# srv902/FOCUS

Measured on AMD Instinct MI355X. Metric: clips/sec (fwd+bwd+opt step) ORViT-MF 16x224, higher is better.
Workload: dtype bf16; 1 GPU; ORViT-Motionformer 16x224, 4 objects, batch=8 per GPU (BASELINE configs[1]); global_batch=8, frames=16, crop=224, objects=4, parallelism=dp1, optimizer=adamw+clipnorm

## Files before the change

focus_amd/asm_lint.py:

```python
import re
import sys

_REG = re.compile(r"\b([va])(\d+)\b|\b([va])\[(\d+):(\d+)\]")
_VM_LOAD = re.compile(r"^(global_load|buffer_load|flat_load|scratch_load)_")
_EFFECT = re.compile(r"^(global_store|buffer_store|flat_store|scratch_store|ds_write|ds_store|global_atomic|buffer_atomic|flat_atomic|"
                     r"ds_add|ds_max|ds_min|ds_bpermute|ds_permute|v_cmp|v_cmpx|v_readlane|v_readfirstlane)")
_KEEPS = re.compile(r"fmac|_mac_|UNUSED_PRESERVE|op_sel|v_dot\w*c_|v_cvt_scalef32_pk_fp8|v_cvt_pk_fp8|v_cvt_sr_|sdwa|_dpp|v_writelane")
_SREG = re.compile(r"^s(\d+)$|^s\[(\d+):(\d+)\]$")


def _regs(text):
    regs = set()
    for m in _REG.finditer(text):
        if m.group(1) is not None:
            regs.add(int(m.group(2)) + (1000 if m.group(1) == "a" else 0))
        else:
            base = 1000 if m.group(3) == "a" else 0
            regs.update(range(base + int(m.group(4)), base + int(m.group(5)) + 1))
    return regs


def _srange(name):
    m = _SREG.match(name)
    if not m:
        return None
    return (int(m.group(1)),) * 2 if m.group(1) is not None else (int(m.group(2)), int(m.group(3)))


def _kernels(asm_path):
    out, name, body, in_asm, pending = [], None, [], False, None
    with open(asm_path) as f:
        for line in f:
            s = line.strip()
            if name is None:
                if pending is not None and s.startswith("; ScratchSize:"):
                    out.append((pending[0], pending[1], int(s.split(":")[1])))
                    pending = None
                m = re.match(r"^(_Z\w+):", line)
                if m:
                    name, body, in_asm = m.group(1), [], False
                continue
            if s.startswith(";;#ASMSTART"):
                in_asm = True
            elif s.startswith(";;#ASMEND"):
                in_asm = False
            elif s.startswith(".Lfunc_end"):
                pending, name = (name, body), None
            else:
                t = s.split(";", 1)[0].strip()
                if t:
                    body.append((t, in_asm))
    return out


def lint_kernel(body):
    labels = {t[:-1]: i for i, (t, _) in enumerate(body) if t.endswith(":")}
    problems, seen = set(), set()
    work = [(0, (), frozenset(), (), None, True)]
    while work:
        i, queue, poison, consts, vcc, live = work.pop()
        queue, poison, consts = list(queue), set(poison), dict(consts)
        while i < len(body):
            t, in_asm = body[i]
            if t.endswith(":"):
                while queue and not queue[0]:
                    queue.pop(0)
                key = (i, tuple(queue), frozenset(poison), tuple(sorted(consts.items())), vcc, live)
                if key in seen:
                    break
                seen.add(key)
                i += 1
                continue
            if t.startswith("."):
                i += 1
                continue
            parts = t.split(None, 1)
            op, args = parts[0], parts[1] if len(parts) > 1 else ""
            ops = [a.strip() for a in args.split(",")]
            if op == "s_waitcnt":
                m = re.search(r"vmcnt\((\d+)\)", t)
                if m:
                    del queue[:max(0, len(queue) - int(m.group(1)))]
                i += 1
                continue
            if op == "s_branch" or op.startswith("s_cbranch"):
                tgt = args.strip()
                if tgt in labels:
                    taken = {"s_cbranch_vccnz": vcc, "s_cbranch_vccz": None if vcc is None else 1 - vcc,
                             "s_cbranch_execnz": 1 if live else None, "s_cbranch_execz": 0 if live else None}.get(op)
                    if op == "s_branch" or taken == 1:
                        i = labels[tgt]
                        continue
                    if taken is None:
                        work.append((labels[tgt], tuple(queue), frozenset(poison), tuple(consts.items()), vcc, live))
                i += 1
                continue
            if op == "s_endpgm":
                break
            flying = frozenset().union(*queue) if queue else frozenset()
            dirty = flying | poison
            effect = bool(_EFFECT.match(op))
            dst = set() if effect and not op.startswith(("v_cmp", "v_read", "ds_bpermute", "ds_permute")) else _regs(ops[0] if ops else "")
            src = _regs(args) if not dst else _regs(",".join(ops[1:]))
            if op.startswith("v_swap"):
                src |= dst
            if dst & flying:
                problems.add("%s writes %s under a hand-issued load still in flight" % (op, _names(dst & flying)))
            hit = src & dirty
            sdst = bool(ops) and (ops[0].startswith(("s", "vcc", "exec", "m0")) and not ops[0].startswith("src"))
            if hit and (effect or sdst or _VM_LOAD.match(op)):
                problems.add("%s uses %s: %s" % (op, _names(hit), "loaded by hand and still in flight" if hit & flying else
                                                 "derived from a register read while its hand-issued load was in flight"))
            elif hit or (dst & poison and _KEEPS.search(t)):
                poison |= dst
            else:
                poison -= dst
            if _VM_LOAD.match(op):
                lds = "_lds_" in op or re.search(r"\blds\b", args)
                hand = in_asm and not lds
                queue.append(frozenset(dst) if hand else frozenset())
                poison -= dst
                if len(queue) > 96:
                    queue.pop(0)
            d0 = ops[0] if ops else ""
            if d0 == "exec" or "saveexec" in op:
                live = op.startswith("s_or_")
            if op == "s_and_b64" and d0 == "vcc" and "exec" in ops[1:] and any(o in consts for o in ops[1:]):
                vcc = 1 if consts[[o for o in ops[1:] if o in consts][0]] else 0
            else:
                if d0.startswith("vcc") or (op.startswith("v_cmp") and "_e64" not in op):
                    vcc = None
                r = _srange(d0)
                if r:
                    for k in [k for k in consts if _srange(k)[0] <= r[1] and r[0] <= _srange(k)[1]]:
                        del consts[k]
                    if op == "s_mov_b64" and len(ops) > 1 and ops[1] in ("-1", "0"):
                        consts[d0] = int(ops[1])
            i += 1
    return sorted(problems)


def _names(regs):
    return ",".join(("a%d" % (r - 1000)) if r >= 1000 else ("v%d" % r) for r in sorted(regs))


def lint_hand_loads(asm_path):
    problems = []
    for name, body, scratch in _kernels(asm_path):
        if not any(a and _VM_LOAD.match(t.split()[0]) for t, a in body if not t.endswith(":")):
            continue
        if scratch:
            problems.append((name, "scratch %d B/lane" % scratch))
        problems += [(name, p) for p in lint_kernel(body)]
    return problems


if __name__ == "__main__":
    for path in sys.argv[1:]:
        for p in lint_hand_loads(path):
            print("%s: %s" % p)
```

focus_amd/build.py:

```python
import concurrent.futures
import glob
import os
import re
import subprocess
import sys

HERE = os.path.dirname(os.path.abspath(__file__))
CSRC = os.path.join(HERE, "csrc")
OBJ = os.path.join(HERE, "lib", "obj")
LIB = os.path.join(HERE, "lib", "libfocus_amd.so")
HIPCC = os.environ.get("HIPCC", "/opt/rocm/bin/hipcc")
FLAGS = os.environ.get("FOCUS_EXTRA_HIPFLAGS", "").split() + ["--offload-arch=gfx950", "-O3", "-fPIC", "-std=c++17", "-Wno-pass-failed", "-Wall",
         "-Wno-unused-function"]


def _stale(target, deps):
    if not os.path.exists(target):
        return True
    t = os.path.getmtime(target)
    return any(os.path.getmtime(d) > t for d in deps)


def _hand_loads(src):
    with open(src) as f:
        return 'asm volatile("global_load_dword' in f.read()


def _device_asm(src):
    return os.path.join(OBJ, os.path.basename(src).replace(".hip", "-hip-amdgcn-amd-amdhsa-gfx950.s"))


def lint_hand_loads(asm_path):
    from focus_amd import asm_lint
    return asm_lint.lint_hand_loads(asm_path)


def _compile(src, headers):
    obj = os.path.join(OBJ, os.path.basename(src).replace(".hip", ".o"))
    if _stale(obj, [src] + headers):
        extra = ["-save-temps=obj"] if _hand_loads(src) else []
        subprocess.check_call([HIPCC] + FLAGS + extra + ["-c", src, "-o", obj])
    if _hand_loads(src):
        if not os.path.exists(_device_asm(src)):
            os.remove(obj)
            raise RuntimeError("%s issues loads by hand but its device assembly %s is missing: rebuild" % (
                os.path.basename(src), _device_asm(src)))
        bad = lint_hand_loads(_device_asm(src))
        if bad:
            os.remove(obj)
            raise RuntimeError("%s: registers of hand-issued loads touched before their wait (%d reports):\n  %s" % (
                os.path.basename(src), len(bad), "\n  ".join("%s: %s" % b for b in bad[:40])))
    return obj


def source_hash():
    import hashlib
    h = hashlib.sha1()
    for f in sorted(glob.glob(os.path.join(CSRC, "*.hip")) + glob.glob(os.path.join(CSRC, "*.h"))) + [
            os.path.join(HERE, "..", "include", "focus_amd.h")]:
        h.update(os.path.basename(f).encode())
        h.update(open(f, "rb").read())
    return h.hexdigest()[:12]


def _stamp():
    root = os.path.join(HERE, "..")
    head = "nogit"
    try:
        head = subprocess.run(["git", "-C", root, "rev-parse", "--short", "HEAD"], capture_output=True, text=True,
                              check=True).stdout.strip()
        if subprocess.run(["git", "-C", root, "status", "--porcelain", "--", "focus_amd/csrc", "include"],
                          capture_output=True, text=True).stdout.strip():
            head += "-dirty"
    except Exception:
        pass
    with open(os.path.join(HERE, "lib", "BUILD_HEAD"), "w") as f:
        f.write("%s src:%s\n" % (head, source_hash()))


def build(force=False, verbose=True):
    os.makedirs(OBJ, exist_ok=True)
    srcs = sorted(glob.glob(os.path.join(CSRC, "*.hip")))
    headers = sorted(glob.glob(os.path.join(CSRC, "*.h"))) + [os.path.join(HERE, "..", "include", "focus_amd.h")]
    if force:
        for f in glob.glob(os.path.join(OBJ, "*.o")):
            os.remove(f)
    with concurrent.futures.ThreadPoolExecutor(max_workers=min(8, len(srcs))) as ex:
        objs = list(ex.map(lambda s: _compile(s, headers), srcs))
    if _stale(LIB, objs):
        subprocess.check_call([HIPCC, "--offload-arch=gfx950", "-shared", "-fPIC", "-o", LIB] + objs)
    if os.path.isdir(os.path.join(HERE, "..", ".git")):
        _stamp()
    if verbose:
        print("built", LIB)
    return LIB


if __name__ == "__main__":
    build(force="--force" in sys.argv)
```

focus_amd/csrc/gemm_mfma_tn_ws.hip:

```cpp
#include "focus_common.h"
#include "gemm_internal.h"
#include <algorithm>
#include <cstdlib>

namespace {

typedef __attribute__((ext_vector_type(8))) __bf16 bf16x8;
typedef __attribute__((ext_vector_type(4))) short s16x4;
typedef __attribute__((ext_vector_type(4))) float f32x4;
typedef __attribute__((address_space(1))) const void gvoid_t;
typedef __attribute__((address_space(3))) void lvoid_t;
typedef __attribute__((address_space(3))) s16x4 lds_s16x4;

constexpr int BKM = 64;
constexpr int SUB = BKM * 256;
constexpr int NSTAGE = 3, NLOAD = 4;

union Frag { bf16x8 v; s16x4 t[2]; uint32_t u[4]; };

__device__ __forceinline__ int swz(int row) { return ((row & 3) | ((row >> 1) & 4)) << 1; }
__device__ __forceinline__ int toff(int row, int col) {
    return row * 256 + ((((col >> 3)) ^ swz(row)) << 4) + (col & 4) * 2;
}
__device__ __forceinline__ bf16x8 col_frag16(const char* tile, int r0, int c0, int lane) {
    const int i = lane & 15;
    const int row = r0 + (i >> 2), col = c0 + 4 * (i & 3);
    Frag f;
    f.t[0] = __builtin_amdgcn_ds_read_tr16_b64_v4i16((lds_s16x4*)(tile + toff(row, col)));
    f.t[1] = __builtin_amdgcn_ds_read_tr16_b64_v4i16((lds_s16x4*)(tile + toff(row + 4, col)));
    return f.v;
}

struct Unit { int i0, j0, m_begin, nk, valid_last; };

template <int BI, int BJ>
__global__ __launch_bounds__(64 * (BI * BJ / 4096 + NLOAD)) void gemm_tn_ws_kernel(const focus_gemm_desc d, int tiles_i, int tiles_j,
                                                                                  int splits, int m_per_split, float* csum) {
    constexpr int NCONS = BI * BJ / 4096;
    constexpr int WJ = BJ / 64;
    constexpr int NSP = BI / 128, NSQ = BJ / 128, NSUBT = NSP + NSQ;
    constexpr int STAGE = NSUBT * SUB;
    constexpr int PIECES = NSUBT * 16 / NLOAD;
    extern __shared__ __attribute__((aligned(16))) char smem[];

    const int tid = threadIdx.x, lane = tid & 63;
    const int w = __builtin_amdgcn_readfirstlane(tid >> 6);
    const int Mred = d.K;
    const bf16_t* Pm = static_cast<const bf16_t*>(d.A);
    const bf16_t* Qm = static_cast<const bf16_t*>(d.B);
    const int64_t ldp = d.csA, ldq = d.rsB;

    const int tiles = tiles_i * tiles_j, nunits = tiles * splits;
    const int G = gridDim.x, xcd = blockIdx.x & 7, jwg = blockIdx.x >> 3;
    const int gx = (G >> 3) + (xcd < (G & 7) ? 1 : 0);
    const int q = nunits >> 3, r = nunits & 7;
    const int band0 = xcd < r ? xcd * (q + 1) : r * (q + 1) + (xcd - r) * q;
    const int band_n = q + (xcd < r ? 1 : 0);
    const int my_units = jwg < band_n ? (band_n - jwg + gx - 1) / gx : 0;
    if (my_units == 0) return;
    auto unit_of = [&](int i) __attribute__((always_inline)) {
        const int u = band0 + jwg + i * gx;
        const int split = u / tiles, tile = u % tiles;
        Unit t;
        t.i0 = (tile % tiles_i) * BI;
        t.j0 = (tile / tiles_i) * BJ;
        t.m_begin = split * m_per_split;
        const int len = min(Mred, t.m_begin + m_per_split) - t.m_begin;
        t.nk = (len + BKM - 1) / BKM;
        t.valid_last = len - (t.nk - 1) * BKM;
        return t;
    };

    if (w >= NCONS) {
        const int L = w - NCONS;
        const int cpos = lane & 15, rin = lane >> 4;
        Unit cur = unit_of(0);
        int iu = 0, ikt = 0;
        auto issue = [&](int st) __attribute__((always_inline)) {
            char* sp = smem + st * STAGE;
            const int mb = cur.m_begin + ikt * BKM;
#pragma unroll
            for (int g = 0; g < PIECES; ++g) {
                const int sub = g >> 2, pi = g * NLOAD + L, row = (pi & 15) * 4 + rin;
                const int m = min(mb + row, Mred - 1);
                const int ch = cpos ^ swz(row);
                const bf16_t* src;
                if (sub < NSP) src = Pm + (int64_t)m * ldp + min(cur.i0 + sub * 128 + ch * 8, d.M - 8);
                else src = Qm + (int64_t)m * ldq + min(cur.j0 + (sub - NSP) * 128 + ch * 8, d.N - 8);
                __builtin_amdgcn_global_load_lds((gvoid_t*)src, (lvoid_t*)(sp + pi * 1024), 16, 0, 0);
            }
            if (++ikt == cur.nk) { ikt = 0; if (++iu < my_units) cur = unit_of(iu); }
        };
        int total = 0;
        for (int i = 0; i < my_units; ++i) total += unit_of(i).nk;
        issue(0);
        if (total > 1) {
            issue(1);
            asm volatile("s_waitcnt vmcnt(%0)" ::"n"(PIECES) : "memory");
        } else {
            asm volatile("s_waitcnt vmcnt(0)" ::: "memory");
        }
        __builtin_amdgcn_s_barrier();
        int st2 = 2;
        for (int t = 0; t < total; ++t) {
            if (t + 2 < total) {
                issue(st2);
                st2 = st2 == 2 ? 0 : st2 + 1;
                asm volatile("s_waitcnt vmcnt(%0)" ::"n"(PIECES) : "memory");
            } else {
                asm volatile("s_waitcnt vmcnt(0)" ::: "memory");
            }
            __builtin_amdgcn_s_barrier();
        }
        return;
    }

    const int wi = w / WJ, wj = w % WJ;
    const int fr = lane & 15, fq = lane >> 4;
    const int poff = (wi >> 1) * SUB, pcol = (wi & 1) * 64;
    const int qoff = (NSP + (wj >> 1)) * SUB, qcol = (wj & 1) * 64;
    f32x4 acc[4][4];
    constexpr int NA = 4 / WJ;
    f32x4 accb[NA];
    Frag ones;
    ones.u[0] = ones.u[1] = ones.u[2] = ones.u[3] = 0x3F803F80u;
    auto compute = [&](const char* stage, auto masked, int valid, bool cs) __attribute__((always_inline)) {
        const char* sp = stage + poff;
        const char* sq = stage + qoff;
#pragma unroll
        for (int ks = 0; ks < 2; ++ks) {
            bf16x8 fp[4], fqv[4];
#pragma unroll
            for (int a = 0; a < 4; ++a) fp[a] = col_frag16(sp, ks * 32 + 8 * fq, pcol + a * 16, lane);
#pragma unroll
            for (int b = 0; b < 4; ++b) fqv[b] = col_frag16(sq, ks * 32 + 8 * fq, qcol + b * 16, lane);
            if constexpr (decltype(masked)::value) {
                const int left = valid - (ks * 32 + 8 * fq);
#pragma unroll
                for (int a = 0; a < 4; ++a) {
                    Frag f; f.v = fp[a];
#pragma unroll
                    for (int e2 = 0; e2 < 4; ++e2) {
                        const uint32_t keep = (2 * e2 < left ? 0x0000ffffu : 0u) | (2 * e2 + 1 < left ? 0xffff0000u : 0u);
                        f.u[e2] &= keep;
                    }
                    fp[a] = f.v;
                }
            }
#pragma unroll
            for (int a = 0; a < 4; ++a)
#pragma unroll
                for (int b = 0; b < 4; ++b)
                    acc[a][b] = __builtin_amdgcn_mfma_f32_16x16x32_bf16(fqv[b], fp[a], acc[a][b], 0, 0, 0);
            if (cs) {
#pragma unroll
                for (int n = 0; n < NA; ++n) {
                    bf16x8 sel = fp[n];
#pragma unroll
                    for (int j = 1; j < WJ; ++j)
                        if (wj == j) sel = fp[j * NA + n];
                    accb[n] = __builtin_amdgcn_mfma_f32_16x16x32_bf16(ones.v, sel, accb[n], 0, 0, 0);
                }
            }
        }
    };

    __builtin_amdgcn_s_barrier();
    int st = 0;
    for (int cu = 0; cu < my_units; ++cu) {
        const Unit cur = unit_of(cu);
#pragma unroll
        for (int a = 0; a < 4; ++a)
#pragma unroll
            for (int b = 0; b < 4; ++b) acc[a][b] = (f32x4){0.f, 0.f, 0.f, 0.f};
        const int tj = cur.j0 / BJ;
        int cs_in = tj;
#pragma unroll
        for (int n = 0; n < NA; ++n) accb[n] = (f32x4){0.f, 0.f, 0.f, 0.f};
        for (int kt = 0; kt + 1 < cur.nk; ++kt) {
            compute(smem + st * STAGE, std::false_type{}, BKM, csum != nullptr && cs_in == 0);
            cs_in = cs_in == 0 ? tiles_j - 1 : cs_in - 1;
            st = st == 2 ? 0 : st + 1;
            __builtin_amdgcn_s_barrier();
        }
        compute(smem + st * STAGE, std::true_type{}, cur.valid_last, csum != nullptr && cs_in == 0);
        st = st == 2 ? 0 : st + 1;
        __builtin_amdgcn_s_barrier();
        const int split = cur.m_begin / m_per_split;
        if (csum && fq == 0) {
#pragma unroll
            for (int n = 0; n < NA; ++n) {
                const int gi = cur.i0 + wi * 64 + (wj * NA + n) * 16 + fr;
                if (gi < d.M) csum[(int64_t)(split * tiles_j + tj) * d.M + gi] = d.alpha * accb[n][0];
            }
        }
        float* C = d.aux ? static_cast<float*>(d.aux) + (int64_t)split * d.M * d.N : static_cast<float*>(d.C);
        const int64_t ldc = d.aux ? d.N : d.rsC;
#pragma unroll
        for (int a = 0; a < 4; ++a) {
            const int gi = cur.i0 + wi * 64 + a * 16 + fr;
            if (gi >= d.M) continue;
#pragma unroll
            for (int b = 0; b < 4; ++b) {
                const int gj = cur.j0 + wj * 64 + b * 16 + fq * 4;
                if (d.aux) {
                    if (gj < d.N)
                        *reinterpret_cast<float4*>(C + (int64_t)gi * ldc + gj) =
                            make_float4(d.alpha * acc[a][b][0], d.alpha * acc[a][b][1], d.alpha * acc[a][b][2], d.alpha * acc[a][b][3]);
                } else {
#pragma unroll
                    for (int r4 = 0; r4 < 4; ++r4)
                        if (gj + r4 < d.N) atomicAdd(C + (int64_t)gi * ldc + (gj + r4), d.alpha * acc[a][b][r4]);
                }
            }
        }
    }
}

template <int BI, int BJ>
int launch_tn_ws(const focus_gemm_desc& d, const focus_tn_plan& pl, float* csum, hipStream_t s) {
    const size_t lds = (size_t)NSTAGE * (BI / 128 + BJ / 128) * SUB;
    auto k = gemm_tn_ws_kernel<BI, BJ>;
    static bool once = (hipFuncSetAttribute((const void*)k, hipFuncAttributeMaxDynamicSharedMemorySize, lds) == hipSuccess);
    (void)once;
    const int nunits = pl.tiles_i * pl.tiles_j * pl.splits;
    hipLaunchKernelGGL(k, dim3(std::min(nunits, 256)), dim3(64 * (BI * BJ / 4096 + NLOAD)), lds, s, d, pl.tiles_i, pl.tiles_j,
                       pl.splits, pl.m_per_split, csum);
    FOCUS_CHECK_LAUNCH();
    return FOCUS_OK;
}

}

focus_tn_plan focus_gemm_tn_ws_plan(int M, int N, int K) {
    static const bool enabled = !(getenv("FOCUS_GEMM_TN_WS") && atoi(getenv("FOCUS_GEMM_TN_WS")) == 0);
    static const int rounds_env = getenv("FOCUS_GEMM_TN_ROUNDS") ? atoi(getenv("FOCUS_GEMM_TN_ROUNDS")) : 0;
    focus_tn_plan p = {};
    if (!enabled || M < 128 || N < 128 || K < 2048) return p;
    const int64_t pad1 = (int64_t)((M + 255) / 256 * 256) * ((N + 127) / 128 * 128);
    const int64_t pad2 = (int64_t)((M + 127) / 128 * 128) * ((N + 255) / 256 * 256);
    bool wide_i = (M >= N || N % 256 != 0) && M >= 256;
    static const bool pad_rule = !(getenv("FOCUS_GEMM_TN_PAD_RULE") && atoi(getenv("FOCUS_GEMM_TN_PAD_RULE")) == 0);
    if (wide_i && pad_rule && pad2 < pad1 && N < 256) wide_i = false;
    if (!wide_i && N < 256 && !(pad2 < pad1)) return p;
    const int bi = wide_i ? 256 : 128, bj = wide_i ? 128 : 256;
    p.kind = wide_i ? 1 : 2;
    p.tiles_i = (M + bi - 1) / bi;
    p.tiles_j = (N + bj - 1) / bj;
    const int tiles = p.tiles_i * p.tiles_j;
    const int max_splits = std::max(1, K / (4 * BKM));
    const int rounds = rounds_env > 0 ? rounds_env : 1;
    const int best_s = std::min(max_splits, std::max(1, 256 * rounds / tiles));
    p.splits = best_s;
    p.m_per_split = ((K + p.splits - 1) / p.splits + BKM - 1) / BKM * BKM;
    p.splits = (K + p.m_per_split - 1) / p.m_per_split;
    return p;
}

int focus_gemm_mfma_tn_ws(const focus_gemm_desc& d, const focus_tn_plan& pl, float* csum, hipStream_t s) {
    if (pl.kind == 1) return launch_tn_ws<256, 128>(d, pl, csum, s);
    if (pl.kind == 2) return launch_tn_ws<128, 256>(d, pl, csum, s);
    return FOCUS_ERR_SHAPE;
}
```

focus_amd/csrc/gemm_tn_group.hip:

```cpp
#include "focus_common.h"
#include "gemm_internal.h"
#include <algorithm>

namespace {

typedef __attribute__((ext_vector_type(8))) __bf16 bf16x8;
typedef __attribute__((ext_vector_type(4))) short s16x4;
typedef __attribute__((ext_vector_type(4))) float f32x4;
typedef __attribute__((address_space(1))) const void gvoid_t;
typedef __attribute__((address_space(3))) void lvoid_t;
typedef __attribute__((address_space(3))) s16x4 lds_s16x4;

constexpr int BKM = 64;
constexpr int SUB = BKM * 256;
constexpr int NSTAGE = 3, NLOAD = 4;
constexpr int BI = 256, BJ = 128;

union Frag { bf16x8 v; s16x4 t[2]; uint32_t u[4]; };

__device__ __forceinline__ int swz(int row) { return ((row & 3) | ((row >> 1) & 4)) << 1; }
__device__ __forceinline__ int toff(int row, int col) {
    return row * 256 + ((((col >> 3)) ^ swz(row)) << 4) + (col & 4) * 2;
}
__device__ __forceinline__ bf16x8 col_frag16(const char* tile, int r0, int c0, int lane) {
    const int i = lane & 15;
    const int row = r0 + (i >> 2), col = c0 + 4 * (i & 3);
    Frag f;
    f.t[0] = __builtin_amdgcn_ds_read_tr16_b64_v4i16((lds_s16x4*)(tile + toff(row, col)));
    f.t[1] = __builtin_amdgcn_ds_read_tr16_b64_v4i16((lds_s16x4*)(tile + toff(row + 4, col)));
    return f.v;
}

struct Prob {
    const bf16_t* P;
    const bf16_t* Q;
    float* C;
    float* db;
    int64_t ldp, ldq;
    int32_t I, J, Mred, tiles_i, tiles_j, pad_;
};
constexpr int MAXP = 8;
struct GroupArgs { Prob p[MAXP]; int32_t nprob, nunits; };
struct UnitRec { int16_t prob, ti, tj, pad_; };

__global__ __launch_bounds__(64 * (BI * BJ / 4096 + NLOAD)) void gemm_tn_group_kernel(const GroupArgs ga, const UnitRec* __restrict__ units) {
    constexpr int NCONS = BI * BJ / 4096;
    constexpr int WJ = BJ / 64;
    constexpr int NSP = BI / 128, NSQ = BJ / 128, NSUBT = NSP + NSQ;
    constexpr int STAGE = NSUBT * SUB;
    constexpr int PIECES = NSUBT * 16 / NLOAD;
    extern __shared__ __attribute__((aligned(16))) char smem[];

    const int tid = threadIdx.x, lane = tid & 63;
    const int w = __builtin_amdgcn_readfirstlane(tid >> 6);
    const int nunits = ga.nunits;
    const int G = gridDim.x, xcd = blockIdx.x & 7, jwg = blockIdx.x >> 3;
    const int gx = (G >> 3) + (xcd < (G & 7) ? 1 : 0);
    const int q8 = nunits >> 3, r8 = nunits & 7;
    const int band0 = xcd < r8 ? xcd * (q8 + 1) : r8 * (q8 + 1) + (xcd - r8) * q8;
    const int band_n = q8 + (xcd < r8 ? 1 : 0);
    const int my_units = jwg < band_n ? (band_n - jwg + gx - 1) / gx : 0;
    if (my_units == 0) return;

    struct Unit { const bf16_t* P; const bf16_t* Q; float* C; float* db; int64_t ldp, ldq; int I, J, Mred, i0, j0, nk, valid_last, tj; };
    auto unit_of = [&](int i) __attribute__((always_inline)) {
        const UnitRec ur = units[band0 + jwg + i * gx];
        const int pi = __builtin_amdgcn_readfirstlane((int)ur.prob);
        Unit t;
        Prob p = ga.p[0];
#pragma unroll
        for (int k = 1; k < MAXP; ++k)
            if (pi == k) p = ga.p[k];
        t.P = p.P; t.Q = p.Q; t.C = p.C; t.db = p.db; t.ldp = p.ldp; t.ldq = p.ldq; t.I = p.I; t.J = p.J; t.Mred = p.Mred;
        t.i0 = __builtin_amdgcn_readfirstlane((int)ur.ti) * BI;
        t.tj = __builtin_amdgcn_readfirstlane((int)ur.tj);
        t.j0 = t.tj * BJ;
        t.nk = (p.Mred + BKM - 1) / BKM;
        t.valid_last = p.Mred - (t.nk - 1) * BKM;
        return t;
    };

    if (w >= NCONS) {
        const int L = w - NCONS;
        const int cpos = lane & 15, rin = lane >> 4;
        Unit cur = unit_of(0);
        int iu = 0, ikt = 0;
        auto issue = [&](int st) __attribute__((always_inline)) {
            char* sp = smem + st * STAGE;
            const int mb = ikt * BKM;
#pragma unroll
            for (int g = 0; g < PIECES; ++g) {
                const int sub = g >> 2, pi = g * NLOAD + L, row = (pi & 15) * 4 + rin;
                const int m = min(mb + row, cur.Mred - 1);
                const int ch = cpos ^ swz(row);
                const bf16_t* src;
                if (sub < NSP) src = cur.P + (int64_t)m * cur.ldp + min(cur.i0 + sub * 128 + ch * 8, cur.I - 8);
                else src = cur.Q + (int64_t)m * cur.ldq + min(cur.j0 + (sub - NSP) * 128 + ch * 8, cur.J - 8);
                __builtin_amdgcn_global_load_lds((gvoid_t*)src, (lvoid_t*)(sp + pi * 1024), 16, 0, 0);
            }
            if (++ikt == cur.nk) { ikt = 0; if (++iu < my_units) cur = unit_of(iu); }
        };
        int total = 0;
        for (int i = 0; i < my_units; ++i) total += unit_of(i).nk;
        issue(0);
        if (total > 1) {
            issue(1);
            asm volatile("s_waitcnt vmcnt(%0)" ::"n"(PIECES) : "memory");
        } else {
            asm volatile("s_waitcnt vmcnt(0)" ::: "memory");
        }
        __builtin_amdgcn_s_barrier();
        int st2 = 2;
        for (int t = 0; t < total; ++t) {
            if (t + 2 < total) {
                issue(st2);
                st2 = st2 == 2 ? 0 : st2 + 1;
                asm volatile("s_waitcnt vmcnt(%0)" ::"n"(PIECES) : "memory");
            } else {
                asm volatile("s_waitcnt vmcnt(0)" ::: "memory");
            }
            __builtin_amdgcn_s_barrier();
        }
        return;
    }

    const int wi = w / WJ, wj = w % WJ;
    const int fr = lane & 15, fq = lane >> 4;
    const int poff = (wi >> 1) * SUB, pcol = (wi & 1) * 64;
    const int qoff = (NSP + (wj >> 1)) * SUB, qcol = (wj & 1) * 64;
    f32x4 acc[4][4];
    constexpr int NA = 4 / WJ;
    f32x4 accb[NA];
    Frag ones;
    ones.u[0] = ones.u[1] = ones.u[2] = ones.u[3] = 0x3F803F80u;
    auto compute = [&](const char* stage, auto masked, int valid, bool cs) __attribute__((always_inline)) {
        const char* sp = stage + poff;
        const char* sq = stage + qoff;
#pragma unroll
        for (int ks = 0; ks < 2; ++ks) {
            bf16x8 fp[4], fqv[4];
#pragma unroll
            for (int a = 0; a < 4; ++a) fp[a] = col_frag16(sp, ks * 32 + 8 * fq, pcol + a * 16, lane);
#pragma unroll
            for (int b = 0; b < 4; ++b) fqv[b] = col_frag16(sq, ks * 32 + 8 * fq, qcol + b * 16, lane);
            if constexpr (decltype(masked)::value) {
                const int left = valid - (ks * 32 + 8 * fq);
#pragma unroll
                for (int a = 0; a < 4; ++a) {
                    Frag f; f.v = fp[a];
#pragma unroll
                    for (int e2 = 0; e2 < 4; ++e2) {
                        const uint32_t keep = (2 * e2 < left ? 0x0000ffffu : 0u) | (2 * e2 + 1 < left ? 0xffff0000u : 0u);
                        f.u[e2] &= keep;
                    }
                    fp[a] = f.v;
                }
            }
#pragma unroll
            for (int a = 0; a < 4; ++a)
#pragma unroll
                for (int b = 0; b < 4; ++b)
                    acc[a][b] = __builtin_amdgcn_mfma_f32_16x16x32_bf16(fqv[b], fp[a], acc[a][b], 0, 0, 0);
            if (cs) {
#pragma unroll
                for (int n = 0; n < NA; ++n) {
                    bf16x8 sel = fp[n];
#pragma unroll
                    for (int j = 1; j < WJ; ++j)
                        if (wj == j) sel = fp[j * NA + n];
                    accb[n] = __builtin_amdgcn_mfma_f32_16x16x32_bf16(ones.v, sel, accb[n], 0, 0, 0);
                }
            }
        }
    };

    __builtin_amdgcn_s_barrier();
    int st = 0;
    for (int cu = 0; cu < my_units; ++cu) {
        const Unit cur = unit_of(cu);
#pragma unroll
        for (int a = 0; a < 4; ++a)
#pragma unroll
            for (int b = 0; b < 4; ++b) acc[a][b] = (f32x4){0.f, 0.f, 0.f, 0.f};
        const bool want_b = cur.db != nullptr && cur.tj == 0;
#pragma unroll
        for (int n = 0; n < NA; ++n) accb[n] = (f32x4){0.f, 0.f, 0.f, 0.f};
        for (int kt = 0; kt + 1 < cur.nk; ++kt) {
            compute(smem + st * STAGE, std::false_type{}, BKM, want_b);
            st = st == 2 ? 0 : st + 1;
            __builtin_amdgcn_s_barrier();
        }
        compute(smem + st * STAGE, std::true_type{}, cur.valid_last, want_b);
        st = st == 2 ? 0 : st + 1;
        __builtin_amdgcn_s_barrier();
        if (want_b && fq == 0) {
#pragma unroll
            for (int n = 0; n < NA; ++n) {
                const int gi = cur.i0 + wi * 64 + (wj * NA + n) * 16 + fr;
                if (gi < cur.I) cur.db[gi] = accb[n][0];
            }
        }
#pragma unroll
        for (int a = 0; a < 4; ++a) {
            const int gi = cur.i0 + wi * 64 + a * 16 + fr;
            if (gi >= cur.I) continue;
#pragma unroll
            for (int b = 0; b < 4; ++b) {
                const int gj = cur.j0 + wj * 64 + b * 16 + fq * 4;
                if (gj < cur.J)
                    *reinterpret_cast<float4*>(cur.C + (int64_t)gi * cur.J + gj) =
                        make_float4(acc[a][b][0], acc[a][b][1], acc[a][b][2], acc[a][b][3]);
            }
        }
    }
}

}

extern "C" int focus_linear_wgrad_group_units(const focus_wgrad_item* items, int n_items) {
    if (!items || n_items <= 0) return 0;
    int64_t t = 0;
    for (int p = 0; p < n_items; ++p) t += (int64_t)((items[p].N + BI - 1) / BI) * ((items[p].K + BJ - 1) / BJ);
    return t > 0x7fffffff ? -1 : (int)t;
}

extern "C" int focus_linear_wgrad_group_plan(const focus_wgrad_item* items, int n_items, void* host_units, size_t bytes) {
    if (!items || !host_units) return FOCUS_ERR_NULL;
    if (n_items <= 0 || n_items > MAXP) return FOCUS_ERR_SHAPE;
    const int total = focus_linear_wgrad_group_units(items, n_items);
    if (total <= 0 || bytes < (size_t)total * sizeof(UnitRec)) return FOCUS_ERR_WORKSPACE;
    UnitRec* u = static_cast<UnitRec*>(host_units);
    constexpr int BA = 4, BB = 8;
    int n = 0;
    for (int p = 0; p < n_items; ++p) {
        const int ti_n = (items[p].N + BI - 1) / BI, tj_n = (items[p].K + BJ - 1) / BJ;
        for (int bi = 0; bi < ti_n; bi += BA)
            for (int bj = 0; bj < tj_n; bj += BB)
                for (int ti = bi; ti < std::min(bi + BA, ti_n); ++ti)
                    for (int tj = bj; tj < std::min(bj + BB, tj_n); ++tj)
                        u[n++] = UnitRec{(int16_t)p, (int16_t)ti, (int16_t)tj, 0};
    }
    return n == total ? FOCUS_OK : FOCUS_ERR_SHAPE;
}

extern "C" int focus_linear_wgrad_group(const focus_wgrad_item* items, int n_items, const void* dev_units, void* stream) {
    if (!items || !dev_units) return FOCUS_ERR_NULL;
    if (n_items <= 0) return FOCUS_OK;
    if (n_items > MAXP) return FOCUS_ERR_SHAPE;
    GroupArgs ga = {};
    int units = 0;
    for (int p = 0; p < n_items; ++p) {
        const focus_wgrad_item& it = items[p];
        if (!it.dy || !it.x || !it.dw) return FOCUS_ERR_NULL;
        if (it.M <= 0 || it.N < 8 || it.K < 8 || (it.N & 7) || (it.K & 7) || (it.ld_dy & 7) || (it.ld_x & 7)) return FOCUS_ERR_SHAPE;
        if (!focus_aligned(it.dy, 16) || !focus_aligned(it.x, 16) || !focus_aligned(it.dw, 16)) return FOCUS_ERR_ALIGN;
        Prob& q = ga.p[p];
        q.P = static_cast<const bf16_t*>(it.dy); q.Q = static_cast<const bf16_t*>(it.x);
        q.C = it.dw; q.db = it.db; q.ldp = it.ld_dy; q.ldq = it.ld_x;
        q.I = it.N; q.J = it.K; q.Mred = it.M;
        q.tiles_i = (it.N + BI - 1) / BI; q.tiles_j = (it.K + BJ - 1) / BJ; q.pad_ = 0;
        if (q.tiles_i > 32767 || q.tiles_j > 32767) return FOCUS_ERR_SHAPE;
        units += q.tiles_i * q.tiles_j;
    }
    ga.nprob = n_items;
    ga.nunits = units;
    hipStream_t s = static_cast<hipStream_t>(stream);
    const size_t lds = (size_t)NSTAGE * (BI / 128 + BJ / 128) * SUB;
    auto k = gemm_tn_group_kernel;
    static bool once = (hipFuncSetAttribute((const void*)k, hipFuncAttributeMaxDynamicSharedMemorySize, lds) == hipSuccess);
    (void)once;
    hipLaunchKernelGGL(k, dim3(std::min(units, 256)), dim3(64 * (BI * BJ / 4096 + NLOAD)), lds, s, ga,
                       static_cast<const UnitRec*>(dev_units));
    FOCUS_CHECK_LAUNCH();
    return FOCUS_OK;
}
```

Measured before the change: 287.3 clips/s.

## Precompute loader source pointers per unit and specialize TN GEMM k-loop on bias-sum

The producer warps in both TN GEMM kernels now compute per-piece source pointers once per work unit and advance them by a k-stride. Only the last k-step still uses clamped row arithmetic. This removes 64-bit multiplies and min clamps from every global_load_lds issue. The grouped kernel reads the problem table straight from the kernarg segment instead of a select chain over MAXP entries. The consumer k-loop is split into two compile-time variants on whether the column-sum MFMA is needed, and an explicit lgkmcnt wait is added before each barrier. A new asm lint fails the build if vector integer multiplies remain beside the DMA loads outside the marked last step. The costs are extra live pointer registers in the loader and a duplicated k-loop body.

After: 297.6 clips/s (median of 6 runs). 1.04x the previous value.

```diff
diff --git a/focus_amd/asm_lint.py b/focus_amd/asm_lint.py
--- a/focus_amd/asm_lint.py
+++ b/focus_amd/asm_lint.py
@@ -155,7 +155,72 @@
     return problems
 
 
+TN_KERNELS = ("gemm_tn_group_kernel", "gemm_tn_ws_kernel")
+TN_MARKER = "focus-lint: clamped-last-step"
+_VMUL = re.compile(r"^(v_mul_lo_u32|v_mul_lo_i32|v_mul_hi_u32|v_mul_hi_i32|v_mad_u64_u32|v_mad_i64_i32)\b")
+_BLOCK_END = re.compile(r"^(s_branch|s_cbranch\w*|s_endpgm|s_setpc_b64)\b")
+
+
+def _raw_kernels(asm_path):
+    out, name, body, pending = [], None, [], None
+    with open(asm_path) as f:
+        for line in f:
+            s = line.strip()
+            if name is None:
+                if pending is not None and s.startswith("; ScratchSize:"):
+                    out.append((pending[0], pending[1], int(s.split(":")[1])))
+                    pending = None
+                m = re.match(r"^(_Z\w+):", line)
+                if m:
+                    name, body = m.group(1), []
+            elif s.startswith(".Lfunc_end"):
+                pending, name = (name, body), None
+            elif s:
+                body.append(s)
+    return out
+
+
+def lint_tn_loader(asm_path, kernels=TN_KERNELS):
+    problems, found = [], 0
+    for name, body, scratch in _raw_kernels(asm_path):
+        if not any(k in name for k in kernels):
+            continue
+        found += 1
+        if scratch:
+            problems.append((name, "scratch %d B/lane" % scratch))
+        blocks, cur = [], []
+        for s in body:
+            if re.match(r"^[.\w$]+:", s):
+                blocks.append(cur)
+                cur = []
+            cur.append(s)
+            if _BLOCK_END.match(s):
+                blocks.append(cur)
+                cur = []
+        blocks.append(cur)
+        dma = 0
+        for b in blocks:
+            code = [s.split(";", 1)[0].strip() for s in b]
+            loads = sum(c.startswith("global_load_lds_dwordx4") for c in code)
+            if not loads:
+                continue
+            dma += loads
+            muls = [c.split()[0] for c in code if _VMUL.match(c)]
+            if muls and not any(TN_MARKER in s for s in b):
+                label = b[0] if re.match(r"^[.\w$]+:", b[0]) else "(unlabelled)"
+                problems.append((name, "block %s issues %d global_load_lds_dwordx4 beside %d vector integer multiplies (%s)" % (
+                    label.split(":")[0], loads, len(muls), ",".join(sorted(set(muls))))))
+        if not dma:
+            problems.append((name, "no global_load_lds_dwordx4 found: the rule has nothing to check"))
+    if not found:
+        problems.append((asm_path, "none of the kernels %s found" % ", ".join(kernels)))
+    return problems
+
+
 if __name__ == "__main__":
     for path in sys.argv[1:]:
         for p in lint_hand_loads(path):
             print("%s: %s" % p)
+        if any(k in open(path).read() for k in TN_KERNELS):
+            for p in lint_tn_loader(path):
+                print("%s: %s" % p)
diff --git a/focus_amd/build.py b/focus_amd/build.py
--- a/focus_amd/build.py
+++ b/focus_amd/build.py
@@ -26,6 +26,13 @@
         return 'asm volatile("global_load_dword' in f.read()
 
 
+TN_LOADER_FILES = ("gemm_tn_group.hip", "gemm_mfma_tn_ws.hip")
+
+
+def _tn_loader(src):
+    return os.path.basename(src) in TN_LOADER_FILES
+
+
 def _device_asm(src):
     return os.path.join(OBJ, os.path.basename(src).replace(".hip", "-hip-amdgcn-amd-amdhsa-gfx950.s"))
 
@@ -35,11 +42,25 @@
     return asm_lint.lint_hand_loads(asm_path)
 
 
+def lint_tn_loader(asm_path):
+    from focus_amd import asm_lint
+    return asm_lint.lint_tn_loader(asm_path)
+
+
 def _compile(src, headers):
     obj = os.path.join(OBJ, os.path.basename(src).replace(".hip", ".o"))
     if _stale(obj, [src] + headers):
-        extra = ["-save-temps=obj"] if _hand_loads(src) else []
+        extra = ["-save-temps=obj"] if _hand_loads(src) or _tn_loader(src) else []
         subprocess.check_call([HIPCC] + FLAGS + extra + ["-c", src, "-o", obj])
+    if _tn_loader(src):
+        if not os.path.exists(_device_asm(src)):
+            os.remove(obj)
+            raise RuntimeError("%s: its device assembly %s is missing: rebuild" % (os.path.basename(src), _device_asm(src)))
+        bad = lint_tn_loader(_device_asm(src))
+        if bad:
+            os.remove(obj)
+            raise RuntimeError("%s: address arithmetic in the loader K loop or scratch use (%d reports):\n  %s" % (
+                os.path.basename(src), len(bad), "\n  ".join("%s: %s" % b for b in bad[:40])))
     if _hand_loads(src):
         if not os.path.exists(_device_asm(src)):
             os.remove(obj)
diff --git a/focus_amd/csrc/gemm_mfma_tn_ws.hip b/focus_amd/csrc/gemm_mfma_tn_ws.hip
--- a/focus_amd/csrc/gemm_mfma_tn_ws.hip
+++ b/focus_amd/csrc/gemm_mfma_tn_ws.hip
@@ -74,25 +74,43 @@
     if (w >= NCONS) {
         const int L = w - NCONS;
         const int cpos = lane & 15, rin = lane >> 4;
-        Unit cur = unit_of(0);
+        Unit cur;
+        const bf16_t* src[PIECES];
         int iu = 0, ikt = 0;
+        auto setup = [&](int i) __attribute__((always_inline)) {
+            cur = unit_of(i);
+#pragma unroll
+            for (int g = 0; g < PIECES; ++g) {
+                const int sub = g >> 2, pi = g * NLOAD + L, row = (pi & 15) * 4 + rin;
+                const int ch = cpos ^ swz(row);
+                if (sub < NSP) src[g] = Pm + (int64_t)(cur.m_begin + row) * ldp + min(cur.i0 + sub * 128 + ch * 8, d.M - 8);
+                else src[g] = Qm + (int64_t)(cur.m_begin + row) * ldq + min(cur.j0 + (sub - NSP) * 128 + ch * 8, d.N - 8);
+            }
+        };
         auto issue = [&](int st) __attribute__((always_inline)) {
             char* sp = smem + st * STAGE;
-            const int mb = cur.m_begin + ikt * BKM;
-#pragma unroll
-            for (int g = 0; g < PIECES; ++g) {
-                const int sub = g >> 2, pi = g * NLOAD + L, row = (pi & 15) * 4 + rin;
-                const int m = min(mb + row, Mred - 1);
-                const int ch = cpos ^ swz(row);
-                const bf16_t* src;
-                if (sub < NSP) src = Pm + (int64_t)m * ldp + min(cur.i0 + sub * 128 + ch * 8, d.M - 8);
-                else src = Qm + (int64_t)m * ldq + min(cur.j0 + (sub - NSP) * 128 + ch * 8, d.N - 8);
-                __builtin_amdgcn_global_load_lds((gvoid_t*)src, (lvoid_t*)(sp + pi * 1024), 16, 0, 0);
-            }
-            if (++ikt == cur.nk) { ikt = 0; if (++iu < my_units) cur = unit_of(iu); }
+            if (ikt + 1 < cur.nk) {
+                const int64_t kp = (int64_t)ikt * BKM * ldp, kq = (int64_t)ikt * BKM * ldq;
+#pragma unroll
+                for (int g = 0; g < PIECES; ++g)
+                    __builtin_amdgcn_global_load_lds((gvoid_t*)(src[g] + ((g >> 2) < NSP ? kp : kq)),
+                                                     (lvoid_t*)(sp + (g * NLOAD + L) * 1024), 16, 0, 0);
+            } else {
+                asm volatile("; focus-lint: clamped-last-step" ::: "memory");
+                const int mb = cur.m_begin + ikt * BKM;
+#pragma unroll
+                for (int g = 0; g < PIECES; ++g) {
+                    const int pi = g * NLOAD + L, row = (pi & 15) * 4 + rin;
+                    const int back = min(mb + row, Mred - 1) - (cur.m_begin + row);
+                    __builtin_amdgcn_global_load_lds((gvoid_t*)(src[g] + (int64_t)back * ((g >> 2) < NSP ? ldp : ldq)),
+                                                     (lvoid_t*)(sp + pi * 1024), 16, 0, 0);
+                }
+            }
+            if (++ikt == cur.nk) { ikt = 0; if (++iu < my_units) setup(iu); }
         };
         int total = 0;
         for (int i = 0; i < my_units; ++i) total += unit_of(i).nk;
+        setup(0);
         issue(0);
         if (total > 1) {
             issue(1);
@@ -124,7 +142,7 @@
     f32x4 accb[NA];
     Frag ones;
     ones.u[0] = ones.u[1] = ones.u[2] = ones.u[3] = 0x3F803F80u;
-    auto compute = [&](const char* stage, auto masked, int valid, bool cs) __attribute__((always_inline)) {
+    auto compute = [&](const char* stage, auto masked, int valid, auto has_cs, bool cs) __attribute__((always_inline)) {
         const char* sp = stage + poff;
         const char* sq = stage + qoff;
 #pragma unroll
@@ -152,7 +170,7 @@
 #pragma unroll
                 for (int b = 0; b < 4; ++b)
                     acc[a][b] = __builtin_amdgcn_mfma_f32_16x16x32_bf16(fqv[b], fp[a], acc[a][b], 0, 0, 0);
-            if (cs) {
+            if (decltype(has_cs)::value && cs) {
 #pragma unroll
                 for (int n = 0; n < NA; ++n) {
                     bf16x8 sel = fp[n];
@@ -177,15 +195,21 @@
         int cs_in = tj;
 #pragma unroll
         for (int n = 0; n < NA; ++n) accb[n] = (f32x4){0.f, 0.f, 0.f, 0.f};
-        for (int kt = 0; kt + 1 < cur.nk; ++kt) {
-            compute(smem + st * STAGE, std::false_type{}, BKM, csum != nullptr && cs_in == 0);
-            cs_in = cs_in == 0 ? tiles_j - 1 : cs_in - 1;
+        auto k_loop = [&](auto has_cs) __attribute__((always_inline)) {
+            for (int kt = 0; kt + 1 < cur.nk; ++kt) {
+                compute(smem + st * STAGE, std::false_type{}, BKM, has_cs, cs_in == 0);
+                cs_in = cs_in == 0 ? tiles_j - 1 : cs_in - 1;
+                st = st == 2 ? 0 : st + 1;
+                asm volatile("s_waitcnt lgkmcnt(0)" ::: "memory");
+                __builtin_amdgcn_s_barrier();
+            }
+            compute(smem + st * STAGE, std::true_type{}, cur.valid_last, has_cs, cs_in == 0);
             st = st == 2 ? 0 : st + 1;
+            asm volatile("s_waitcnt lgkmcnt(0)" ::: "memory");
             __builtin_amdgcn_s_barrier();
-        }
-        compute(smem + st * STAGE, std::true_type{}, cur.valid_last, csum != nullptr && cs_in == 0);
-        st = st == 2 ? 0 : st + 1;
-        __builtin_amdgcn_s_barrier();
+        };
+        if (csum) k_loop(std::true_type{});
+        else k_loop(std::false_type{});
         const int split = cur.m_begin / m_per_split;
         if (csum && fq == 0) {
 #pragma unroll
diff --git a/focus_amd/csrc/gemm_tn_group.hip b/focus_amd/csrc/gemm_tn_group.hip
--- a/focus_amd/csrc/gemm_tn_group.hip
+++ b/focus_amd/csrc/gemm_tn_group.hip
@@ -1,6 +1,7 @@
 #include "focus_common.h"
 #include "gemm_internal.h"
 #include <algorithm>
+#include <cstddef>
 
 namespace {
 
@@ -62,46 +63,63 @@
     const int my_units = jwg < band_n ? (band_n - jwg + gx - 1) / gx : 0;
     if (my_units == 0) return;
 
+    static_assert(offsetof(GroupArgs, p) == 0, "the problem table opens the kernel-argument segment");
+    typedef __attribute__((address_space(4))) const Prob cprob_t;
+    cprob_t* tab = (cprob_t*)__builtin_amdgcn_kernarg_segment_ptr();
     struct Unit { const bf16_t* P; const bf16_t* Q; float* C; float* db; int64_t ldp, ldq; int I, J, Mred, i0, j0, nk, valid_last, tj; };
     auto unit_of = [&](int i) __attribute__((always_inline)) {
         const UnitRec ur = units[band0 + jwg + i * gx];
-        const int pi = __builtin_amdgcn_readfirstlane((int)ur.prob);
+        cprob_t* p = tab + __builtin_amdgcn_readfirstlane((int)ur.prob);
         Unit t;
-        Prob p = ga.p[0];
-#pragma unroll
-        for (int k = 1; k < MAXP; ++k)
-            if (pi == k) p = ga.p[k];
-        t.P = p.P; t.Q = p.Q; t.C = p.C; t.db = p.db; t.ldp = p.ldp; t.ldq = p.ldq; t.I = p.I; t.J = p.J; t.Mred = p.Mred;
+        t.P = p->P; t.Q = p->Q; t.C = p->C; t.db = p->db; t.ldp = p->ldp; t.ldq = p->ldq; t.I = p->I; t.J = p->J; t.Mred = p->Mred;
         t.i0 = __builtin_amdgcn_readfirstlane((int)ur.ti) * BI;
         t.tj = __builtin_amdgcn_readfirstlane((int)ur.tj);
         t.j0 = t.tj * BJ;
-        t.nk = (p.Mred + BKM - 1) / BKM;
-        t.valid_last = p.Mred - (t.nk - 1) * BKM;
+        t.nk = (t.Mred + BKM - 1) / BKM;
+        t.valid_last = t.Mred - (t.nk - 1) * BKM;
         return t;
     };
 
     if (w >= NCONS) {
         const int L = w - NCONS;
         const int cpos = lane & 15, rin = lane >> 4;
-        Unit cur = unit_of(0);
+        Unit cur;
+        const bf16_t* src[PIECES];
         int iu = 0, ikt = 0;
+        auto setup = [&](int i) __attribute__((always_inline)) {
+            cur = unit_of(i);
+#pragma unroll
+            for (int g = 0; g < PIECES; ++g) {
+                const int sub = g >> 2, pi = g * NLOAD + L, row = (pi & 15) * 4 + rin;
+                const int ch = cpos ^ swz(row);
+                if (sub < NSP) src[g] = cur.P + (int64_t)row * cur.ldp + min(cur.i0 + sub * 128 + ch * 8, cur.I - 8);
+                else src[g] = cur.Q + (int64_t)row * cur.ldq + min(cur.j0 + (sub - NSP) * 128 + ch * 8, cur.J - 8);
+            }
+        };
         auto issue = [&](int st) __attribute__((always_inline)) {
             char* sp = smem + st * STAGE;
-            const int mb = ikt * BKM;
-#pragma unroll
-            for (int g = 0; g < PIECES; ++g) {
-                const int sub = g >> 2, pi = g * NLOAD + L, row = (pi & 15) * 4 + rin;
-                const int m = min(mb + row, cur.Mred - 1);
-                const int ch = cpos ^ swz(row);
-                const bf16_t* src;
-                if (sub < NSP) src = cur.P + (int64_t)m * cur.ldp + min(cur.i0 + sub * 128 + ch * 8, cur.I - 8);
-                else src = cur.Q + (int64_t)m * cur.ldq + min(cur.j0 + (sub - NSP) * 128 + ch * 8, cur.J - 8);
-                __builtin_amdgcn_global_load_lds((gvoid_t*)src, (lvoid_t*)(sp + pi * 1024), 16, 0, 0);
-            }
-            if (++ikt == cur.nk) { ikt = 0; if (++iu < my_units) cur = unit_of(iu); }
+            if (ikt + 1 < cur.nk) {
+                const int64_t kp = (int64_t)ikt * BKM * cur.ldp, kq = (int64_t)ikt * BKM * cur.ldq;
+#pragma unroll
+                for (int g = 0; g < PIECES; ++g)
+                    __builtin_amdgcn_global_load_lds((gvoid_t*)(src[g] + ((g >> 2) < NSP ? kp : kq)),
+                                                     (lvoid_t*)(sp + (g * NLOAD + L) * 1024), 16, 0, 0);
+            } else {
+                asm volatile("; focus-lint: clamped-last-step" ::: "memory");
+                const int mb = ikt * BKM;
+#pragma unroll
+                for (int g = 0; g < PIECES; ++g) {
+                    const int pi = g * NLOAD + L, row = (pi & 15) * 4 + rin;
+                    const int back = min(mb + row, cur.Mred - 1) - row;
+                    __builtin_amdgcn_global_load_lds((gvoid_t*)(src[g] + (int64_t)back * ((g >> 2) < NSP ? cur.ldp : cur.ldq)),
+                                                     (lvoid_t*)(sp + pi * 1024), 16, 0, 0);
+                }
+            }
+            if (++ikt == cur.nk) { ikt = 0; if (++iu < my_units) setup(iu); }
         };
         int total = 0;
         for (int i = 0; i < my_units; ++i) total += unit_of(i).nk;
+        setup(0);
         issue(0);
         if (total > 1) {
             issue(1);
@@ -133,7 +151,7 @@
     f32x4 accb[NA];
     Frag ones;
     ones.u[0] = ones.u[1] = ones.u[2] = ones.u[3] = 0x3F803F80u;
-    auto compute = [&](const char* stage, auto masked, int valid, bool cs) __attribute__((always_inline)) {
+    auto compute = [&](const char* stage, auto masked, int valid, auto cs) __attribute__((always_inline)) {
         const char* sp = stage + poff;
         const char* sq = stage + qoff;
 #pragma unroll
@@ -161,7 +179,7 @@
 #pragma unroll
                 for (int b = 0; b < 4; ++b)
                     acc[a][b] = __builtin_amdgcn_mfma_f32_16x16x32_bf16(fqv[b], fp[a], acc[a][b], 0, 0, 0);
-            if (cs) {
+            if constexpr (decltype(cs)::value) {
 #pragma unroll
                 for (int n = 0; n < NA; ++n) {
                     bf16x8 sel = fp[n];
@@ -185,14 +203,20 @@
         const bool want_b = cur.db != nullptr && cur.tj == 0;
 #pragma unroll
         for (int n = 0; n < NA; ++n) accb[n] = (f32x4){0.f, 0.f, 0.f, 0.f};
-        for (int kt = 0; kt + 1 < cur.nk; ++kt) {
-            compute(smem + st * STAGE, std::false_type{}, BKM, want_b);
+        auto k_loop = [&](auto cs) __attribute__((always_inline)) {
+            for (int kt = 0; kt + 1 < cur.nk; ++kt) {
+                compute(smem + st * STAGE, std::false_type{}, BKM, cs);
+                st = st == 2 ? 0 : st + 1;
+                asm volatile("s_waitcnt lgkmcnt(0)" ::: "memory");
+                __builtin_amdgcn_s_barrier();
+            }
+            compute(smem + st * STAGE, std::true_type{}, cur.valid_last, cs);
             st = st == 2 ? 0 : st + 1;
+            asm volatile("s_waitcnt lgkmcnt(0)" ::: "memory");
             __builtin_amdgcn_s_barrier();
-        }
-        compute(smem + st * STAGE, std::true_type{}, cur.valid_last, want_b);
-        st = st == 2 ? 0 : st + 1;
-        __builtin_amdgcn_s_barrier();
+        };
+        if (want_b) k_loop(std::true_type{});
+        else k_loop(std::false_type{});
         if (want_b && fq == 0) {
 #pragma unroll
             for (int n = 0; n < NA; ++n) {
```
